# 6Lackiu/EMplanner_Carla

Measured on AMD Instinct MI355X. Metric: planning cycles/sec (DP+QP, 40x9 S-L lattice, 8 obs), higher is better.
Workload: dtype f64

## Files before the change

### emplanner_carla_amd/csrc/emp_frenet_core.h

```cpp
#pragma once

#include "emp_core.h"

namespace emp {

struct Node {
    double x, y, theta, kappa;
};
EMP_HD Node node_at(const double* line, int i) { return Node{line[4 * i], line[4 * i + 1], line[4 * i + 2], line[4 * i + 3]}; }

EMP_HD int match_scan(const double* line, int n_ref, double x, double y, int first, int step, int limit) {
    int match = 0, worse = 0;
    double best = __builtin_inf();
    for (int i = first; i >= 0 && i < n_ref; i += step) {
        const double dx = line[4 * i] - x, dy = line[4 * i + 1] - y;
        const double d = sqrt(dx * dx + dy * dy);
        if (d < best) {
            best = d;
            match = i;
            worse = 0;
        } else if (++worse >= limit) {
            break;
        }
    }
    return match;
}

EMP_HD double dot2(double a0, double a1, double b0, double b1) { return __builtin_fma(a1, b1, a0 * b0); }

EMP_HD Node project_on(const Node& m, double x, double y) {
    const double c = cos(m.theta), s = sin(m.theta);
    const double ds = dot2(x - m.x, y - m.y, c, s);
    return Node{m.x + ds * c, m.y + ds * s, m.theta + m.kappa * ds, m.kappa};
}

EMP_HD Node project_on_cs(const Node& m, double c, double s, double x, double y) {
    const double ds = dot2(x - m.x, y - m.y, c, s);
    return Node{m.x + ds * c, m.y + ds * s, m.theta + m.kappa * ds, m.kappa};
}
EMP_HD double projection_s_cs(const Node& m, double c, double s, double s_at_m, double x, double y) {
    return s_at_m + dot2(x - m.x, y - m.y, c, s);
}

EMP_HD double projection_s(const Node& m, double s_at_m, double x, double y) {
    return s_at_m + dot2(x - m.x, y - m.y, cos(m.theta), sin(m.theta));
}

EMP_HD double lateral_offset(const Node& proj, double x, double y) {
    return dot2(x - proj.x, y - proj.y, -sin(proj.theta), cos(proj.theta));
}

EMP_HD void s_map_build(const double* line, int n_ref, double ox, double oy, double* s_map) {
    const int m0 = match_scan(line, n_ref, ox, oy, 0, 1, 50);
    double acc = 0.0;
    s_map[0] = 0.0;
    for (int i = 1; i < n_ref; ++i) {
        const double dx = line[4 * i] - line[4 * (i - 1)], dy = line[4 * i + 1] - line[4 * (i - 1) + 1];
        acc = sqrt(dx * dx + dy * dy) + acc;
        s_map[i] = acc;
    }
    const double s0 = projection_s(node_at(line, m0), s_map[m0], ox, oy);
    for (int i = 0; i < n_ref; ++i) s_map[i] = s_map[i] - s0;
}

struct FrenetState {
    double l, l_dot, s_dot, l_ddot, dl_ds, s_ddot, ddl_ds;
};
EMP_HD FrenetState frenet_state(const Node& proj, double px, double py, double vx, double vy, double ax, double ay) {
    FrenetState o;
    const double c = cos(proj.theta), s = sin(proj.theta);
    const double k = proj.kappa;
    o.l = dot2(px - proj.x, py - proj.y, -s, c);
    o.l_dot = dot2(vx, vy, -s, c);
    o.s_dot = dot2(vx, vy, c, s) / (1.0 - k * o.l);
    o.l_ddot = dot2(ax, ay, -s, c) - k * (1.0 - k * o.l) * (o.s_dot * o.s_dot);
    o.dl_ds = (fabs(o.s_dot) < 1e-6) ? 0.0 : o.l_dot / o.s_dot;
    o.s_ddot = (dot2(ax, ay, c, s) + 2.0 * (o.s_dot * o.s_dot * k * o.dl_ds) + o.s_dot * o.s_dot * 0.0 * o.l) / (1.0 - k * o.l);
    o.ddl_ds = (fabs(o.s_dot) < 1e-6) ? 0.0 : (o.l_ddot - o.dl_ds * o.s_ddot) / (o.s_dot * o.s_dot);
    return o;
}

EMP_HD bool proj_point(const double* line, const double* s_map, int n_ref, double s, int* idx, Node* out) {
    int i = *idx;
    while (true) {
        if (i + 1 >= n_ref) return false;
        if (!(s_map[i + 1] < s)) break;
        ++i;
    }
    const Node m = node_at(line, i);
    const double ds = s - s_map[i];
    *out = Node{m.x + ds * cos(m.theta), m.y + ds * sin(m.theta), m.theta + m.kappa * ds, m.kappa};
    *idx = i;
    return true;
}

EMP_HD void heading_kappa(const double* xy, int stride, int m, double* theta, int tstride, double* kappa, int kstride) {
    for (int i = 0; i < m; ++i) {
        const int a = (i - 1 > 0) ? i - 1 : 0, b = (i < m - 2) ? i : m - 2;
        const double dx = ((xy[(a + 1) * stride] - xy[a * stride]) + (xy[(b + 1) * stride] - xy[b * stride])) / 2.0;
        const double dy = ((xy[(a + 1) * stride + 1] - xy[a * stride + 1]) + (xy[(b + 1) * stride + 1] - xy[b * stride + 1])) / 2.0;
        theta[i * tstride] = atan2(dy, dx);
    }
    for (int i = 0; i < m; ++i) {
        const int a = (i - 1 > 0) ? i - 1 : 0, b = (i < m - 2) ? i : m - 2;
        const double dx = ((xy[(a + 1) * stride] - xy[a * stride]) + (xy[(b + 1) * stride] - xy[b * stride])) / 2.0;
        const double dy = ((xy[(a + 1) * stride + 1] - xy[a * stride + 1]) + (xy[(b + 1) * stride + 1] - xy[b * stride + 1])) / 2.0;
        const double dpre = theta[(a + 1) * tstride] - theta[a * tstride];
        const double daft = theta[(b + 1) * tstride] - theta[b * tstride];
        kappa[i * kstride] = sin((dpre + daft) / 2.0) / sqrt(dx * dx + dy * dy);
    }
}

}
```

### emplanner_carla_amd/csrc/emp_tail_kernels.h

```cpp
#pragma once

#include <hip/hip_runtime.h>

#include "emp_core.h"
#include "emp_frenet_core.h"
#include "emp_qp_core.h"
#include "emp_qp_wave.h"
#include "emp_qp_rows.h"
#include "emp_smooth_rows.h"

namespace emp {

constexpr int kStDpInfeasible = 1, kStSOutOfRange = 2, kStBoundIndex = 4, kStQpFailed = 8, kStSmoothFailed = 16,
              kStTruncated = 32;

struct QpDev {
    PathQpParams qp;
    double obs_length, obs_width;
    int decimate, midpoint, use_qp;
    int debug_stage;
};

template <int CTRL, int ROW_MASK>
__device__ __forceinline__ void prefix_min_step(double& d, int& li) {
// ... 31 lines not shown
    const int lane = threadIdx.x & 63;
    double d = __builtin_inf();
    if (lane < P) {
        const double dx = lx[lane] - x, dy = ly[lane] - y;
        d = sqrt(dx * dx + dy * dy);
    }
    double pm = d;
    pm = prefix_fmin_step<0x111, 0xF>(pm);
    pm = prefix_fmin_step<0x112, 0xF>(pm);
    pm = prefix_fmin_step<0x114, 0xF>(pm);
    pm = prefix_fmin_step<0x118, 0xF>(pm);
    pm = prefix_fmin_step<0x142, 0xA>(pm);
    pm = prefix_fmin_step<0x143, 0xC>(pm);
    const double back = __shfl(pm, lane >= limit ? lane - limit : 0, 64);
    const unsigned long long stop = __ballot(lane < P && lane >= limit && pm == back);
    const int last = stop ? __builtin_ffsll((long long)stop) - 1 : P - 1;
    const double target = __shfl(pm, last, 64);
    const unsigned long long hit = __ballot(lane <= last && d == target);
    return hit ? __builtin_ffsll((long long)hit) - 1 : 0;
}

__device__ inline int match_scan_wave(const double* lx, const double* ly, int P, double x, double y, int limit) {
    if (P <= 64 && limit >= 1) return match_scan_wave64(lx, ly, P, x, y, limit);
    const int lane = threadIdx.x & 63;
    double cd = __builtin_inf();
    int ci = 0;
    for (int base = 0; base < P; base += 64) {
        const int i = base + lane;
        double d = __builtin_inf();
        int li = i;
        if (i < P) {
            const double dx = lx[i] - x, dy = ly[i] - y;
            d = sqrt(dx * dx + dy * dy);
        }
        prefix_min_first(d, li);
        if (!(d < cd)) {
            d = cd;
            li = ci;
        }
        const unsigned long long stop = __ballot(i < P && i - li >= limit);
        if (stop) {
            const int first = __builtin_ffsll((long long)stop) - 1;
            return __shfl(li, first, 64);
        }
        const int last = min(63, P - 1 - base);
        cd = __shfl(d, last, 64);
        ci = __shfl(li, last, 64);
    }
    return ci;
}

__global__ __launch_bounds__(64) void frenet_project_wave_kernel(
    int B, int max_ref, int max_obs, const double* __restrict__ ref_line, const int* __restrict__ n_ref,
    const double* __restrict__ origin_xy, const double* __restrict__ start_xy, const double* __restrict__ start_v,
    const double* __restrict__ start_a, const double* __restrict__ obs_xy, const int* __restrict__ n_obs,
    double* __restrict__ s_map, double* __restrict__ obs_s, double* __restrict__ obs_l, double* __restrict__ begin_sl,
    double* __restrict__ start, int obs_cap, const double* __restrict__ dyn, int* __restrict__ n_obs_out) {
    __builtin_amdgcn_s_setprio(EMP_PRIO_FRONT);
    extern __shared__ __attribute__((aligned(16))) double lds[];
    const int b = blockIdx.x, lane = threadIdx.x & 63;
    double* lx = lds;
    double* ly = lx + max_ref;
    double* lth = ly + max_ref;
    double* lk = lth + max_ref;
    double* sm = lk + max_ref;
    double* lcos = sm + max_ref;
    double* lsin = lcos + max_ref;
    const double* line = ref_line + (size_t)b * max_ref * 4;
    const int P = min(max(n_ref[b], 0), max_ref);
    const int k = n_obs ? min(max(n_obs[b], 0), max_obs) : 0;
    const double ox = origin_xy[2 * b], oy = origin_xy[2 * b + 1];
    const double px = start_xy[2 * b], py = start_xy[2 * b + 1];
    double obx = 0.0, oby = 0.0;
    if (lane < k) {
        obx = obs_xy[((size_t)b * max_obs + lane) * 2];
        oby = obs_xy[((size_t)b * max_obs + lane) * 2 + 1];
    }
    for (int i = lane; i < P; i += 64) {
        lx[i] = line[4 * i];
        ly[i] = line[4 * i + 1];
        const double th = line[4 * i + 2];
        lth[i] = th;
        lk[i] = line[4 * i + 3];
        lcos[i] = cos(th);
        lsin[i] = sin(th);
    }
    if (P == 0 && lane == 0) {
        lx[0] = ly[0] = lth[0] = lk[0] = sm[0] = lsin[0] = 0.0;
        lcos[0] = 1.0;
    }
    __syncthreads();
    double carry = 0.0;
    for (int base = 0; base < P; base += 64) {
        const int i = base + lane;
        double d = 0.0;
        if (i >= 1 && i < P) {
            const double dx = lx[i] - lx[i - 1], dy = ly[i] - ly[i - 1];
            d = sqrt(dx * dx + dy * dy);
        }
        const int cnt = min(64, P - base);
        if (lane == 0) d = (base >= 1) ? d + carry : 0.0;
        double mine = d;
        for (int k = 1; k < cnt; ++k) mine = d + lane_up1(mine);
        carry = __shfl(mine, cnt - 1, 64);
        if (i < P) sm[i] = mine;
    }
    __syncthreads();
    auto node = [&](int i) { return Node{lx[i], ly[i], lth[i], lk[i]}; };
    const int m0 = match_scan_wave(lx, ly, P, ox, oy, 50);
    const double s0 = projection_s_cs(node(m0), lcos[m0], lsin[m0], sm[m0], ox, oy);
    __syncthreads();
    for (int i = lane; i < P; i += 64) {
        const double v = sm[i] - s0;
        sm[i] = v;
        s_map[(size_t)b * max_ref + i] = v;
    }
    __syncthreads();
    int my_match = 0, first_match = 0;
    for (int j = 0; j < k; ++j) {
        if (j >= 64 && (j & 63) == 0 && (j & ~63) + lane < k) {
            obx = obs_xy[((size_t)b * max_obs + (j & ~63) + lane) * 2];
            oby = obs_xy[((size_t)b * max_obs + (j & ~63) + lane) * 2 + 1];
        }
        const double x = __shfl(obx, j & 63, 64), y = __shfl(oby, j & 63, 64);
        const int mj = match_scan_wave(lx, ly, P, x, y, 50);
        if (j == 0) first_match = mj;
        if ((j & 63) == lane) my_match = mj;
        if ((j & 63) == 63 || j == k - 1) {
            const int jj = (j & ~63) + lane;
            if (jj <= j) {
                obs_s[(size_t)b * obs_cap + jj] = projection_s_cs(node(my_match), lcos[my_match], lsin[my_match], sm[my_match], obx, oby);
                obs_l[(size_t)b * obs_cap + jj] = lateral_offset(project_on_cs(node(first_match), lcos[first_match], lsin[first_match], obx, oby), obx, oby);
            }
        }
    }
    const int ms = match_scan_wave(lx, ly, P, px, py, 50);
    if (lane == 0) {
        const Node proj = project_on_cs(node(ms), lcos[ms], lsin[ms], px, py);
        const double bs = projection_s_cs(node(ms), lcos[ms], lsin[ms], sm[ms], px, py);
        if (begin_sl) {
            begin_sl[2 * b] = bs;
            begin_sl[2 * b + 1] = lateral_offset(proj, px, py);
        }
        const FrenetState fs = frenet_state(proj, px, py, start_v[2 * b], start_v[2 * b + 1], start_a[2 * b], start_a[2 * b + 1]);
        start[4 * b + 0] = bs;
        start[4 * b + 1] = fs.l;
        start[4 * b + 2] = fs.dl_ds;
        start[4 * b + 3] = fs.ddl_ds;
        int total = k;
        if (dyn && !isnan(dyn[2 * b]) && k + 3 <= obs_cap) {
            const double Len_vehicle = 2.910, Len_obs = 3.0;
            const double Dis = dyn[2 * b], V_obs = dyn[2 * b + 1];
            const double vx = start_v[2 * b], vy = start_v[2 * b + 1];
            const double V_ego = sqrt(vx * vx + vy * vy);
            const double delta_v = V_ego - V_obs;
            const double meet_t = ((Dis - Len_vehicle / 2.0) - Len_obs / 2.0) / delta_v;
            const double delta_t = (Len_vehicle + Len_obs) / delta_v;
            const double leave_t = meet_t + delta_t;
            const double meet_s = ((bs + Dis) + V_obs * meet_t) - Len_obs / 2.0;
            const double leave_s = ((bs + Dis) + V_obs * leave_t) + Len_obs / 2.0;
            const double delta_s = leave_s - meet_s;
            const double obs_pos = meet_s + delta_s / 2.0;
            if (leave_s < 80.0) {
                double* os = obs_s + (size_t)b * obs_cap + k;
                double* ol = obs_l + (size_t)b * obs_cap + k;
                os[0] = meet_s - 10.0;
                os[1] = obs_pos;
                os[2] = leave_s;
                ol[0] = ol[1] = ol[2] = 0.0;
                total = k + 3;
            }
        }
        if (n_obs_out) n_obs_out[b] = total;
    }
}

__device__ inline int find_match_one(const double* line, int P, double x, double y, bool windowed, int st) {
    if (!windowed) return match_scan(line, P, x, y, 0, 1, 50);
    const Node pm = node_at(line, st);
    const double flag = dot2(x - pm.x, y - pm.y, cos(pm.theta), sin(pm.theta));
    return match_scan(line, P, x, y, st, flag > 0.0 ? 1 : -1, 5);
}

__global__ void match_points_kernel(int B, int max_ref, int max_pts, const double* __restrict__ ref_line,
                                    const int* __restrict__ n_ref, const double* __restrict__ xy,
                                    const int* __restrict__ n_pts, const int* __restrict__ is_first_run,
                                    const int* __restrict__ pre_match_index, int* __restrict__ match_index,
                                    double* __restrict__ proj, int windowed_api) {
    const int b = blockIdx.x * blockDim.x + threadIdx.x;
    if (b >= B) return;
    const double* line = ref_line + (size_t)b * max_ref * 4;
    const int P = min(max(n_ref[b], 0), max_ref);
    const int k = min(max(n_pts[b], 0), max_pts);
    int m_first = 0;
    const bool windowed = windowed_api && !is_first_run[b];
    if (P < 1 || (windowed && (pre_match_index[b] < 0 || pre_match_index[b] >= P))) {
        for (int j = 0; j < k; ++j) {
            match_index[(size_t)b * max_pts + j] = -1;
            double* o = proj + ((size_t)b * max_pts + j) * 4;
            o[0] = o[1] = o[2] = o[3] = __builtin_nan("");
        }
        return;
    }
    for (int j = 0; j < k; ++j) {
        const double x = xy[((size_t)b * max_pts + j) * 2], y = xy[((size_t)b * max_pts + j) * 2 + 1];
        const int m = find_match_one(line, P, x, y, windowed, windowed ? pre_match_index[b] : 0);
        if (j == 0) m_first = m;
        match_index[(size_t)b * max_pts + j] = m;
        const Node pr = project_on(node_at(line, m_first), x, y);
        double* o = proj + ((size_t)b * max_pts + j) * 4;
        o[0] = pr.x;
        o[1] = pr.y;
        o[2] = pr.theta;
        o[3] = pr.kappa;
    }
}

__global__ void heading_kappa_kernel(int B, int max_pts, const double* __restrict__ xy, const int* __restrict__ n_pts,
                                     double* __restrict__ theta, double* __restrict__ kappa) {
    const int b = blockIdx.x * blockDim.x + threadIdx.x;
    if (b >= B) return;
    const int m = min(max(n_pts[b], 0), max_pts);
    if (m < 2) return;
    heading_kappa(xy + (size_t)b * max_pts * 2, 2, m, theta + (size_t)b * max_pts, 1, kappa + (size_t)b * max_pts, 1);
}

__device__ inline int argmin_abs(const double* s, int stride, int n, double target) {
    int best = 0;
    double bv = fabs(s[0] - target);
    for (int j = 1; j < n; ++j) {
        const double v = fabs(s[j * stride] - target);
        if (v < bv) {
            bv = v;
            best = j;
        }
    }
    return best;
}

__device__ inline void argmin_abs3(const double* s, int n, double t0, double t1, double t2, int* i0, int* i1, int* i2) {
    const double f = s[0];
    double b0 = fabs(f - t0), b1 = fabs(f - t1), b2 = fabs(f - t2);
    int k0 = 0, k1 = 0, k2 = 0;
    for (int j0 = 1; j0 < n; j0 += 4) {
        double v[4];
#pragma unroll
        for (int u = 0; u < 4; ++u) v[u] = s[min(j0 + u, n - 1)];
#pragma unroll
        for (int u = 0; u < 4; ++u) {
            const int j = j0 + u;
            const double a0 = fabs(v[u] - t0), a1 = fabs(v[u] - t1), a2 = fabs(v[u] - t2);
            if (a0 < b0) { b0 = a0; k0 = j; }
            if (a1 < b1) { b1 = a1; k1 = j; }
            if (a2 < b2) { b2 = a2; k2 = j; }
        }
    }
// ... 101 lines not shown
        status[b] = rc ? kStSmoothFailed : 0;
    }
}

constexpr int kRefLinePoints = 51;

__global__ __launch_bounds__(64) void reference_line_wave_kernel(int B, int max_global, SmoothQpParams sx, SmoothQpParams sy,
                                                                 const double* __restrict__ global_path,
                                                                 const int* __restrict__ n_global,
                                                                 const double* __restrict__ pred_xy,
                                                                 const int* __restrict__ is_first_run,
                                                                 const int* __restrict__ pre_match_index,
                                                                 double* __restrict__ ref_line, int* __restrict__ n_ref,
                                                                 int* __restrict__ match_index, int* __restrict__ iters,
                                                                 int* __restrict__ status, int n_ref_on_fail = 0) {
    extern __shared__ __attribute__((aligned(16))) double lds[];
    const int b = blockIdx.x, lane = threadIdx.x & 63;
    const double* line = global_path + (size_t)b * max_global * 4;
    const int P = min(n_global[b], max_global);
    double* gxy = lds;
    double* qmem = gxy + 2 * kRefLinePoints;
    double* out = ref_line + (size_t)b * kRefLinePoints * 4;
    int m = 0, first = 0, fail = 0;
    if (lane == 0) {
        const double x = pred_xy[2 * b], y = pred_xy[2 * b + 1];
        const int st = pre_match_index[b];
        if (P < 1 || ((!is_first_run || !is_first_run[b]) && (st < 0 || st >= P))) {
            fail = kStSOutOfRange;
        } else if (is_first_run && is_first_run[b]) {
            m = match_scan(line, P, x, y, 0, 1, 50);
        } else {
            const Node pm = node_at(line, st);
            const double flag = dot2(x - pm.x, y - pm.y, cos(pm.theta), sin(pm.theta));
            m = match_scan(line, P, x, y, st, flag > 0.0 ? 1 : -1, 5);
        }
        int back = 10, fwd = 40;
        if (m < back) {
            back = m;
            fwd = 50 - back;
        }
        if (P - m - 1 < fwd) {
            fwd = P - m - 1;
            back = 50 - fwd;
        }
        first = m - back;
        if (!fail && (first < 0 || m + fwd + 1 > P)) fail = kStSOutOfRange;
    }
    m = __shfl(m, 0, 64);
    first = __shfl(first, 0, 64);
    fail = __shfl(fail, 0, 64);
    int it = 0;
    if (!fail) {
        if (lane < kRefLinePoints) {
            gxy[2 * lane] = line[4 * (first + lane)];
            gxy[2 * lane + 1] = line[4 * (first + lane) + 1];
        }
        __syncthreads();
        double *px = nullptr, *py = nullptr;
        const int rc = smooth_pair_wave<true>(qmem, gxy, 2, kRefLinePoints, sx, sy, &px, &py, &it);
        if (rc) fail = kStSmoothFailed;
        else heading_kappa_wave(px, py, kRefLinePoints, qmem + 2 * BoxRangeQp::words(kRefLinePoints, kRefLinePoints), out, 4);
    }
    if (fail)
        for (int i = lane; i < kRefLinePoints * 4; i += 64) out[i] = 0.0;
    if (lane == 0) {
        n_ref[b] = fail ? n_ref_on_fail : kRefLinePoints;
        match_index[b] = m;
        if (iters) iters[b] = it;
        status[b] = fail;
    }
}

__device__ inline int frenet_path_to_xy(const double* line, const double* s_map, int P, double begin_s, double begin_l,
                                        const double* path_s, const double* path_l, int n, double* target_xy,
                                        int cap, bool* s_error, bool* trunc) {
    *s_error = false;
    *trunc = false;
    int idx = 0, m = 0;
    Node pr;
    if (!proj_point(line, s_map, P, begin_s, &idx, &pr)) {
        *s_error = true;
        return 0;
    }
    target_xy[0] = pr.x + begin_l * (-sin(pr.theta));
    target_xy[1] = pr.y + begin_l * cos(pr.theta);
    m = 1;
    for (int i = 0; i < n; ++i) {
        const double s = path_s[i];
        if (s > s_map[P - 1]) break;
        if (!proj_point(line, s_map, P, s, &idx, &pr)) {
            *s_error = true;
            return m;
        }
        if (m >= cap) {
            *trunc = true;
            break;
        }
        target_xy[2 * m] = pr.x + path_l[i] * (-sin(pr.theta));
        target_xy[2 * m + 1] = pr.y + path_l[i] * cos(pr.theta);
        ++m;
    }
    return m;
}

__global__ void path_to_xy_kernel(int B, int max_ref, int max_pts, const double* __restrict__ ref_line,
                                  const double* __restrict__ s_map, const int* __restrict__ n_ref,
                                  const double* __restrict__ begin_sl, const double* __restrict__ path_s,
                                  const double* __restrict__ path_l, const int* __restrict__ n_pts,
                                  double* __restrict__ target_xy, int* __restrict__ n_out, int* __restrict__ status) {
    const int b = blockIdx.x * blockDim.x + threadIdx.x;
    if (b >= B) return;
    const int P = min(max(n_ref[b], 0), max_ref);
    const int n = min(max(n_pts[b], 0), max_pts);
    bool s_err, trunc;
    const int m = frenet_path_to_xy(ref_line + (size_t)b * max_ref * 4, s_map + (size_t)b * max_ref, P,
                                    begin_sl[2 * b], begin_sl[2 * b + 1], path_s + (size_t)b * max_pts,
                                    path_l + (size_t)b * max_pts, n, target_xy + (size_t)b * (max_pts + 1) * 2,
                                    max_pts + 1, &s_err, &trunc);
    n_out[b] = m;
    status[b] = (s_err ? kStSOutOfRange : 0) | (trunc ? kStTruncated : 0);
}

template <int G, int R = 0>
__host__ __device__ constexpr int cycle_qp_group_words(int cap, int max_obs) {
    if (R > 0) return PathQpRowsLayout<(R > 0 ? G : 8), (R > 0 ? R : 3)>::stride(max_obs);
    return 5 * cap + 4 * max_obs + (G == 32 ? path_qp_words_pair() : path_qp_words(cap));
}
template <int G, int R = 0>
__device__ __forceinline__ void cycle_qp_body(int B, int max_pts, int max_obs, int cap, const QpDev& Q,
                                                           const double* __restrict__ dp_s,
                                                           const double* __restrict__ dp_l,
                                                           const int* __restrict__ dp_len,
                                                           const double* __restrict__ obs_s,
                                                           const double* __restrict__ obs_l,
                                                           const int* __restrict__ n_obs,
                                                           const double* __restrict__ start,
                                                           double* __restrict__ path_s, double* __restrict__ path_l,
                                                           int* __restrict__ path_len, int* __restrict__ status) {
    extern __shared__ __attribute__((aligned(16))) double lds_all[];
    __builtin_amdgcn_s_setprio(EMP_PRIO_BACK);
    constexpr int GPW = 64 / G;
    const int lane = threadIdx.x & 63, grp = lane / G, gl = lane & (G - 1);
    const int b = blockIdx.x * GPW + grp;
    const bool present = b < B;
    static_assert(R == 0 || G == 8 || G == 16, "the rows solver runs on groups of 8 or 16 lanes");
    const int per_group = cycle_qp_group_words<G, R>(cap, max_obs);
    double* lds = lds_all + (size_t)grp * per_group;
    const size_t o = (size_t)(present ? b : 0) * max_pts;
    double* sd = lds;
    double *ld, *lmin, *lmax, *ql, *otab, *qmem;
    if constexpr (R > 0) {
        using L = PathQpRowsLayout<G, R>;
        qmem = lds;
        ql = qmem + L::result;
        sd = qmem + L::path;
        ld = sd + cap;
        lmin = ld + cap;
        lmax = lmin + cap;
        otab = qmem + (max_obs <= L::C ? L::obstacles : L::words);
    } else {
        ld = sd + cap;
        lmin = ld + cap;
        lmax = lmin + cap;
        ql = lmax + cap;
        otab = ql + cap;
        qmem = otab + 4 * max_obs;
    }
#ifdef EMP_QP_PROBE_EMPTY
    if (Q.debug_stage == 4) return;
#endif
    const int ne = present ? dp_len[b] : 0;
    const int dec = Q.decimate > 0 ? Q.decimate : 1;
    const int n = (ne + dec - 1) / dec;
    const int st = present ? status[b] : 0;
    int fail = 0;
    if (present && (n > cap || n + (Q.midpoint ? 1 : 0) > max_pts || n < 1)) fail = kStTruncated;
    bool live = present && !fail;
    for (int i = gl; i < (live ? n : 0); i += G) {
        sd[i] = dp_s[o + (size_t)i * dec];
        ld[i] = dp_l[o + (size_t)i * dec];
    }
    __syncthreads();
// ... 103 lines not shown
                    }
                }
                plen = n + 1;
            } else {
                for (int i = gl; i < n; i += G) {
                    ps[i] = sd_at(i);
                    pl[i] = ql[i];
                }
                plen = n;
            }
        }
        for (int i = plen + gl; i < max_pts; i += G) {
            ps[i] = 0.0;
            pl[i] = 0.0;
        }
        if (gl == 0) {
            path_len[b] = plen;
            status[b] = st | fail;
        }
    }
}

#define EMP_CYCLE_QP_PARAMS                                                                                         \
    int B, int max_pts, int max_obs, int cap, QpDev Q, const double *__restrict__ dp_s, const double *__restrict__ dp_l, \
        const int *__restrict__ dp_len, const double *__restrict__ obs_s, const double *__restrict__ obs_l,           \
        const int *__restrict__ n_obs, const double *__restrict__ start, double *__restrict__ path_s,                  \
        double *__restrict__ path_l, int *__restrict__ path_len, int *__restrict__ status
#define EMP_CYCLE_QP_ARGS B, max_pts, max_obs, cap, Q, dp_s, dp_l, dp_len, obs_s, obs_l, n_obs, start, path_s, path_l, path_len, status
template <int G>
__global__ __launch_bounds__(64) void cycle_qp_wave_kernel(EMP_CYCLE_QP_PARAMS) {
    cycle_qp_body<G>(EMP_CYCLE_QP_ARGS);
}
template <int GP, int R>
__global__ __launch_bounds__(64) void cycle_qp_rows_kernel(EMP_CYCLE_QP_PARAMS) {
    cycle_qp_body<GP, R>(EMP_CYCLE_QP_ARGS);
}
#undef EMP_CYCLE_QP_PARAMS
#undef EMP_CYCLE_QP_ARGS

__device__ inline int walk_from_zero(const double* sm, int P, double s, bool* off_end) {
    int lo = 0, hi = P - 1;
    while (lo < hi) {
        const int mid = (lo + hi) >> 1;
        if (sm[mid + 1] < s) lo = mid + 1;
        else hi = mid;
    }
    *off_end = lo + 1 >= P;
    return lo;
}

template <bool WIDE>
__device__ __forceinline__ void cycle_cartesian_body(
    int B, int max_ref, int max_pts, int cap, SmoothQpParams sx, SmoothQpParams sy, const double* __restrict__ ref_line,
    const double* __restrict__ s_map, const int* __restrict__ n_ref, const double* __restrict__ begin_sl,
    const double* __restrict__ path_s, const double* __restrict__ path_l, const int* __restrict__ path_len,
    double* __restrict__ traj, int* __restrict__ traj_len, int* __restrict__ status) {
    extern __shared__ __attribute__((aligned(16))) double lds[];
    __builtin_amdgcn_s_setprio(EMP_PRIO_CART);
    const int b = blockIdx.x, lane = threadIdx.x & 63;
    double* sm = lds;
    double* txy = sm + max_ref;
    double* th = txy + 2 * cap;
    double* qmem = th + cap;
    const int st = status[b];
    double* out_rows = traj + (size_t)b * (max_pts + 1) * 4;
    auto body = [&]() -> int {
    const double* line = ref_line + (size_t)b * max_ref * 4;
    const int P = min(max(n_ref[b], 0), max_ref);
    const int n = path_len[b];
    for (int i = lane; i < P; i += 64) sm[i] = s_map[(size_t)b * max_ref + i];
    __syncthreads();
    bool off = false;
    const double bs = begin_sl[2 * b], bl = begin_sl[2 * b + 1];
    const int idx0 = walk_from_zero(sm, P, bs, &off);
    if (off || P < 2) {
        if (lane == 0) status[b] = st | kStSOutOfRange;
        return 0;
    }
    if (st & (kStQpFailed | kStBoundIndex | kStTruncated)) return 0;
    if (lane == 0) {
        const Node m0 = node_at(line, idx0);
        const double ds = bs - sm[idx0];
        const double th0 = m0.theta + m0.kappa * ds;
        txy[0] = (m0.x + ds * cos(m0.theta)) + bl * (-sin(th0));
        txy[1] = (m0.y + ds * sin(m0.theta)) + bl * cos(th0);
    }
    const double s_last = sm[P - 1];
    int carry = idx0, count = n;
    for (int base = 0; base < n; base += 64) {
        const int i = base + lane;
        const bool in = i < n;
        const double s = in ? path_s[(size_t)b * max_pts + i] : 0.0;
        const int first_bad = __builtin_ffsll((long long)__ballot(in && s > s_last));
        if (first_bad) count = min(count, base + first_bad - 1);
        bool o2 = false;
        int k = in ? walk_from_zero(sm, P, fmin(s, s_last), &o2) : 0;
        for (int d = 1; d < 64; d <<= 1) {
            const int v = __shfl_up(k, d, 64);
            if (lane >= d) k = max(k, v);
        }
        k = max(k, carry);
        carry = __shfl(k, 63, 64);
        if (in && i < count && i + 1 < cap) {
            const Node mm = node_at(line, k);
            const double ds = s - sm[k];
            const double thp = mm.theta + mm.kappa * ds;
            const double l = path_l[(size_t)b * max_pts + i];
            txy[2 * (i + 1)] = (mm.x + ds * cos(mm.theta)) + l * (-sin(thp));
            txy[2 * (i + 1) + 1] = (mm.y + ds * sin(mm.theta)) + l * cos(thp);
        }
        if (first_bad) break;
    }
    const int m = count + 1;
    __syncthreads();
    if (m > cap || m > max_pts + 1) {
        if (lane == 0) status[b] = st | kStTruncated;
        return 0;
    }
    if (m < 2) {
        if (lane == 0) status[b] = st | kStSmoothFailed;
        return 0;
    }
    int it = 0;
    double *px = nullptr, *py = nullptr;
    const int rc = smooth_pair_wave<WIDE>(qmem, txy, 2, m, sx, sy, &px, &py, &it);
    if (rc) {
        if (lane == 0) status[b] = st | kStSmoothFailed;
        return 0;
    }
    heading_kappa_wave(px, py, m, th, out_rows, 4);
    return m;
    };
    const int m_out = body();
    for (int i = m_out * 4 + lane; i < (max_pts + 1) * 4; i += 64) out_rows[i] = 0.0;
    if (lane == 0) traj_len[b] = m_out;
}

#define EMP_CARTESIAN_ARGS B, max_ref, max_pts, cap, sx, sy, ref_line, s_map, n_ref, begin_sl, path_s, path_l, path_len, traj, traj_len, status
__global__ __launch_bounds__(64) void cycle_cartesian_wave_kernel_wide(
    int B, int max_ref, int max_pts, int cap, SmoothQpParams sx, SmoothQpParams sy, const double* __restrict__ ref_line,
    const double* __restrict__ s_map, const int* __restrict__ n_ref, const double* __restrict__ begin_sl,
    const double* __restrict__ path_s, const double* __restrict__ path_l, const int* __restrict__ path_len,
    double* __restrict__ traj, int* __restrict__ traj_len, int* __restrict__ status) {
    cycle_cartesian_body<true>(EMP_CARTESIAN_ARGS);
}
__global__ __launch_bounds__(64) __attribute__((amdgpu_waves_per_eu(4, 4))) void cycle_cartesian_wave_kernel_narrow(
    int B, int max_ref, int max_pts, int cap, SmoothQpParams sx, SmoothQpParams sy, const double* __restrict__ ref_line,
    const double* __restrict__ s_map, const int* __restrict__ n_ref, const double* __restrict__ begin_sl,
    const double* __restrict__ path_s, const double* __restrict__ path_l, const int* __restrict__ path_len,
    double* __restrict__ traj, int* __restrict__ traj_len, int* __restrict__ status) {
    cycle_cartesian_body<false>(EMP_CARTESIAN_ARGS);
}
#undef EMP_CARTESIAN_ARGS

template <int GP, int R>
__global__ __launch_bounds__(64) void cycle_cartesian_rows_kernel(
    int B, int max_ref, int max_pts, int cap, SmoothQpParams sx, SmoothQpParams sy, const double* __restrict__ ref_line,
    const double* __restrict__ s_map, const int* __restrict__ n_ref, const double* __restrict__ begin_sl,
    const double* __restrict__ path_s, const double* __restrict__ path_l, const int* __restrict__ path_len,
    double* __restrict__ traj, int* __restrict__ traj_len, int* __restrict__ status, int force_fallback) {
    extern __shared__ __attribute__((aligned(16))) double lds[];
    __builtin_amdgcn_s_setprio(EMP_PRIO_CART);
    constexpr int SL = 2 * GP, SPW = 64 / SL;
    const int lane = threadIdx.x & 63, sc = lane / SL, sl = lane & (SL - 1);
    const int b = blockIdx.x * SPW + sc;
    const bool present = b < B;
    const size_t bb = present ? (size_t)b : 0;
    const int per_scene = max_ref + 5 * cap;
    double* sm = lds + (size_t)sc * per_scene;
    double* txy = sm + max_ref;
    double* th = txy + 2 * cap;
    double* px = th + cap;
    double* py = px + cap;
    double* qmem = lds + (size_t)SPW * per_scene;
    const int st = present ? status[bb] : 0;
    int add = 0;
    bool alive = present && !(st & (kStQpFailed | kStBoundIndex | kStTruncated));
    const double* line = ref_line + bb * max_ref * 4;
    const int P = present ? min(max(n_ref[bb], 0), max_ref) : 0;
    const int n = alive ? path_len[bb] : 0;
    for (int i = sl; i < P; i += SL) sm[i] = s_map[bb * max_ref + i];
    __syncthreads();
    bool off = false;
    const double bs = present ? begin_sl[2 * bb] : 0.0, bl = alive ? begin_sl[2 * bb + 1] : 0.0;
    const int idx0 = walk_from_zero(sm, P, bs, &off);
    if (present && (off || P < 2)) {
        add = kStSOutOfRange;
        alive = false;
    }
    if (alive && sl == 0) {
        const Node m0 = node_at(line, idx0);
        const double ds = bs - sm[idx0];
        const double th0 = m0.theta + m0.kappa * ds;
        txy[0] = (m0.x + ds * cos(m0.theta)) + bl * (-sin(th0));
        txy[1] = (m0.y + ds * sin(m0.theta)) + bl * cos(th0);
    }
    const double s_last = alive ? sm[P - 1] : 0.0;
    int carry = idx0, count = alive ? n : 0;
    bool stop = !alive;
    int nmax = 0;
#pragma unroll
    for (int g = 0; g < SPW; ++g) nmax = max(nmax, __builtin_amdgcn_readlane(alive ? n : 0, SL * g));
    constexpr unsigned long long kSceneMask = (SL == 32) ? 0xffffffffull : 0xffffull;
    for (int base = 0; base < nmax; base += SL) {
        const int i = base + sl;
        const bool in = !stop && i < n;
        const double s = in ? path_s[bb * max_pts + i] : 0.0;
        const unsigned bad16 = (unsigned)((__ballot(in && s > s_last) >> (SL * sc)) & kSceneMask);
        const int first_bad = __builtin_ffs((int)bad16);
        if (!stop && first_bad) count = min(count, base + first_bad - 1);
        bool o2 = false;
        int k = in ? walk_from_zero(sm, P, fmin(s, s_last), &o2) : 0;
        for (int d = 1; d < SL; d <<= 1) {
            const int v = __shfl_up(k, d, SL);
            if (sl >= d) k = max(k, v);
        }
        k = max(k, carry);
        carry = __shfl(k, SL - 1, SL);
        if (in && i < count && i + 1 < cap) {
            const Node mm = node_at(line, k);
            const double ds = s - sm[k];
            const double thp = mm.theta + mm.kappa * ds;
            const double l = path_l[bb * max_pts + i];
            txy[2 * (i + 1)] = (mm.x + ds * cos(mm.theta)) + l * (-sin(thp));
            txy[2 * (i + 1) + 1] = (mm.y + ds * sin(mm.theta)) + l * cos(thp);
        }
        if (first_bad) stop = true;
    }
    int m = count + 1;
    __syncthreads();
    if (alive && (m > cap || m > max_pts + 1 || m > GP * R)) {
        add = kStTruncated;
        alive = false;
    }
    if (alive && m < 2) {
        add = kStSmoothFailed;
        alive = false;
    }
    const int grp = sl / GP, gl = sl & (GP - 1);
    double ref[R], u[R];
#pragma unroll
    for (int r = 0; r < R; ++r) {
        const int j = gl * R + r;
        const double v = txy[2 * (j < cap ? j : 0) + grp];
        ref[r] = (alive && j < m) ? v : 0.0;
    }
    int it = 0;
    int rc = box_qp_active_set_rows<GP, R>(ref, alive ? m : 0, grp ? sy : sx, u, &it);
    if (force_fallback && rc == 0) rc = -1;
    const unsigned long long unsettled = __ballot(alive && rc < 0), wrong = __ballot(alive && rc > 0);
    const bool need_fb = ((unsettled >> (SL * sc)) & kSceneMask) != 0ull;
    if (((wrong >> (SL * sc)) & kSceneMask) != 0ull) {
        add = kStSmoothFailed;
        alive = false;
    }
    if (alive && !need_fb) {
#pragma unroll
        for (int r = 0; r < R; ++r) {
            const int j = gl * R + r;
            if (j < m) (grp ? py : px)[j] = u[r];
        }
    }
    __syncthreads();
    if (unsettled != 0ull) {
        for (int s2 = 0; s2 < SPW; ++s2) {
            if (((unsettled >> (SL * s2)) & kSceneMask) == 0ull) continue;
            const int m2 = __builtin_amdgcn_readlane(m, SL * s2);
            double* base2 = lds + (size_t)s2 * per_scene;
            double *qx = nullptr, *qy = nullptr;
            int it2 = 0;
            const int rc2 = smooth_pair_wave<(GP * R > 32)>(qmem, base2 + max_ref, 2, m2, sx, sy, &qx, &qy, &it2);
            if (rc2 == 0) {
                for (int i = lane; i < m2; i += 64) {
                    base2[max_ref + 3 * cap + i] = qx[i];
                    base2[max_ref + 4 * cap + i] = qy[i];
                }
            } else if (sc == s2) {
                add = kStSmoothFailed;
                alive = false;
            }
            __syncthreads();
        }
    }
    double* out_rows = traj + bb * (max_pts + 1) * 4;
    const int mm = alive ? m : 0;
    for (int i = sl; i < mm; i += SL) {
        const int a = (i - 1 > 0) ? i - 1 : 0, c = (i < mm - 2) ? i : mm - 2;
        const double dx = ((px[a + 1] - px[a]) + (px[c + 1] - px[c])) / 2.0;
        const double dy = ((py[a + 1] - py[a]) + (py[c + 1] - py[c])) / 2.0;
        th[i] = atan2(dy, dx);
    }
    __syncthreads();
    for (int i = sl; i < mm; i += SL) {
        const int a = (i - 1 > 0) ? i - 1 : 0, c = (i < mm - 2) ? i : mm - 2;
        const double dx = ((px[a + 1] - px[a]) + (px[c + 1] - px[c])) / 2.0;
        const double dy = ((py[a + 1] - py[a]) + (py[c + 1] - py[c])) / 2.0;
        const double dpre = th[a + 1] - th[a], daft = th[c + 1] - th[c];
        double* o = out_rows + (size_t)i * 4;
        o[0] = px[i];
        o[1] = py[i];
        o[2] = th[i];
        o[3] = sin((dpre + daft) / 2.0) / sqrt(dx * dx + dy * dy);
    }
    if (present) {
        for (int i = mm * 4 + sl; i < (max_pts + 1) * 4; i += SL) out_rows[i] = 0.0;
        if (sl == 0) {
            traj_len[bb] = mm;
            if (add) status[bb] = st | add;
// ... 54 lines not shown
    int m_first = 0;
    for (int j = 0; j < k; ++j) {
        const size_t o = (size_t)b * max_pts + j;
        double* r = out + o * 7;
        if (P < 1) {
            r[0] = r[1] = r[2] = r[3] = r[4] = r[5] = r[6] = __builtin_nan("");
            continue;
        }
        const double x = xy[o * 2], y = xy[o * 2 + 1];
        const int m = match_scan(line, P, x, y, 0, 1, 50);
        if (j == 0) m_first = m;
        const Node proj = project_on(node_at(line, m_first), x, y);
        const FrenetState f = frenet_state(proj, origin_xy[2 * b], origin_xy[2 * b + 1], vxy[o * 2], vxy[o * 2 + 1],
                                           axy[o * 2], axy[o * 2 + 1]);
        r[0] = f.l; r[1] = f.l_dot; r[2] = f.s_dot; r[3] = f.l_ddot; r[4] = f.dl_ds; r[5] = f.s_ddot; r[6] = f.ddl_ds;
    }
}

__global__ void proj_point_kernel(int n, int max_ref, const double* __restrict__ ref_line,
                                  const double* __restrict__ s_map, const int* __restrict__ n_ref,
                                  const double* __restrict__ s, const int* __restrict__ pre_idx,
                                  double* __restrict__ out, int* __restrict__ idx_out, int* __restrict__ status) {
    const int t = blockIdx.x * blockDim.x + threadIdx.x;
    if (t >= n) return;
    const int P = min(max(n_ref[t], 0), max_ref);
    int idx = pre_idx[t];
    Node pr{0, 0, 0, 0};
    const bool ok = idx >= 0 && proj_point(ref_line + (size_t)t * max_ref * 4, s_map + (size_t)t * max_ref, P, s[t], &idx, &pr);
    out[4 * t] = pr.x; out[4 * t + 1] = pr.y; out[4 * t + 2] = pr.theta; out[4 * t + 3] = pr.kappa;
    idx_out[t] = idx;
    status[t] = ok ? 0 : kStSOutOfRange;
}

__device__ inline double chord_length(double x0, double y0, double x1, double y1) {
    const double dx = x1 - x0, dy = y1 - y0;
    return sqrt(dx * dx + dy * dy);
}

__global__ void index2s_kernel(int B, int max_pts, const double* __restrict__ x, const double* __restrict__ y,
                               const int* __restrict__ n_pts, double* __restrict__ out) {
    const int b = blockIdx.x * blockDim.x + threadIdx.x;
    if (b >= B) return;
    const size_t o = (size_t)b * max_pts;
    const int n = min(max(n_pts[b], 0), max_pts);
    double acc = 0.0;
    for (int i = 0; i < n; ++i) out[o + i] = 0.0;
    for (int i = 1; i < n; ++i) {
        if (x[o + i] != x[o + i]) break;
        acc += chord_length(x[o + i - 1], y[o + i - 1], x[o + i], y[o + i]);
        out[o + i] = acc;
    }
}

__global__ void frenet2cartesian_kernel(int B, int max_ref, int max_pts, const double* __restrict__ ref_line,
                                        const double* __restrict__ index2s, const int* __restrict__ n_ref,
                                        const double* __restrict__ sl, const int* __restrict__ n_pts,
                                        double* __restrict__ out, int* __restrict__ status, int proj_only) {
    const int b = blockIdx.x * blockDim.x + threadIdx.x;
    if (b >= B) return;
    const double* line = ref_line + (size_t)b * max_ref * 4;
    const double* sm = index2s + (size_t)b * max_ref;
    const int P = min(max(n_ref[b], 0), max_ref);
    const int k = min(max(n_pts[b], 0), max_pts);
    const double qnan = __builtin_nan("");
    int st = 0;
    bool stopped = false;
    for (int j = 0; j < k; ++j) {
        const double* v = sl + ((size_t)b * max_pts + j) * 4;
        double* o = out + ((size_t)b * max_pts + j) * 4;
        o[0] = o[1] = o[2] = o[3] = qnan;
        if (stopped || v[0] != v[0]) {
            stopped = true;
            continue;
        }
        int idx = 1;
        while (idx < P && sm[idx] < v[0]) ++idx;
        if (idx >= P) {
            st = kStSOutOfRange;
            stopped = true;
            continue;
        }
        const Node m = node_at(line, idx);
        const double ds = v[0] - sm[idx];
        const double px = m.x + ds * cos(m.theta), py = m.y + ds * sin(m.theta);
        const double ph = m.theta + ds * m.kappa, pk = m.kappa;
        if (proj_only) {
            o[0] = px; o[1] = py; o[2] = ph; o[3] = pk;
            continue;
        }
        const double l = v[1], dl = v[2], ddl = v[3];
        o[0] = px + l * (-sin(ph));
        o[1] = py + l * cos(ph);
        const double hd = ph + atan(dl / (1.0 - pk * l));
        const double dth = hd - ph;
        o[2] = hd;
        o[3] = ((ddl + pk * dl * tan(dth)) * (cos(dth) * cos(dth)) / (1.0 - pk * l) + pk) * cos(dth) / (1.0 - pk * l);
    }
    status[b] = st;
}

__device__ inline void dy_obs_deri_one(double l, double vx, double vy, double hd, double k, double* s_dot_out, double* l_dot_out,
                                       double* dl_out) {
    const double l_dot = dot2(vx, vy, -sin(hd), cos(hd));
    const double s_dot = dot2(vx, vy, cos(hd), sin(hd)) / (1.0 - k * l);
    *s_dot_out = s_dot;
    *l_dot_out = l_dot;
    *dl_out = (fabs(s_dot) < 1e-6) ? 0.0 : l_dot / s_dot;
}

__global__ void dy_obs_deri_kernel(int n, const double* __restrict__ in, double* __restrict__ out) {
    const int t = blockIdx.x * blockDim.x + threadIdx.x;
    if (t >= n) return;
    dy_obs_deri_one(in[5 * t], in[5 * t + 1], in[5 * t + 2], in[5 * t + 3], in[5 * t + 4], &out[3 * t], &out[3 * t + 1], &out[3 * t + 2]);
}

__global__ void quintic_kernel(int n, const double* __restrict__ bc, double* __restrict__ coeff) {
    const int t = blockIdx.x * blockDim.x + threadIdx.x;
    if (t >= n) return;
    const double* v = bc + 8 * t;
    const double l0 = v[0], dl0 = v[1], ddl0 = v[2], l1 = v[3], dl1 = v[4], ddl1 = v[5], s0 = v[6], T = v[7] - v[6];
    const double h = l1 - l0, T2 = T * T, T3 = T2 * T, T4 = T3 * T, T5 = T4 * T;
    double a[6];
    a[0] = l0;
    a[1] = dl0;
    a[2] = 0.5 * ddl0;
    a[3] = (20.0 * h - (8.0 * dl1 + 12.0 * dl0) * T - (3.0 * ddl0 - ddl1) * T2) / (2.0 * T3);
    a[4] = (-30.0 * h + (14.0 * dl1 + 16.0 * dl0) * T + (3.0 * ddl0 - 2.0 * ddl1) * T2) / (2.0 * T4);
    a[5] = (12.0 * h - 6.0 * (dl1 + dl0) * T - (ddl0 - ddl1) * T2) / (2.0 * T5);
    double c[6] = {a[5], 0, 0, 0, 0, 0};
    int deg = 0;
    for (int k = 4; k >= 0; --k) {
        ++deg;
        for (int j = deg; j >= 1; --j) c[j] = c[j - 1] - s0 * c[j];
        c[0] = a[k] - s0 * c[0];
    }
    for (int j = 0; j < 6; ++j) coeff[6 * t + j] = c[j];
}

__global__ void obs_cost_kernel(int n, int samples, double w, double danger, double safe, const double* __restrict__ sq,
                                double* __restrict__ cost) {
    const int t = blockIdx.x * blockDim.x + threadIdx.x;
    if (t >= n) return;
    const double d2a = danger * danger, d2b = safe * safe;
    double c = 0.0;
    for (int i = 0; i < samples; ++i) {
        const double v = sq[(size_t)samples * t + i];
        if (v <= d2a) {
            c = c + w;
            break;
        } else if (d2a < v && v < d2b) {
            c = c + kSoftGain / v;
        }
    }
    cost[t] = c;
}

__global__ void free_edge_cost_kernel(int n, int max_obs, const double* __restrict__ edges, const double* __restrict__ obs_s,
                                      const double* __restrict__ obs_l, const int* __restrict__ n_obs, double w_coll, double w0,
                                      double w1, double w2, double w_ref, double* __restrict__ cost) {
    const int t = blockIdx.x * blockDim.x + threadIdx.x;
    if (t >= n) return;
    const double* e = edges + (size_t)t * 8;
    const Quintic q = quintic_shifted(e[1], e[2], e[3], e[5], e[4]);
    const int k = max_obs > 0 ? min(max(n_obs[t], 0), max_obs) : 0;
    cost[t] = segment_cost(q, e[0], e[6], obs_s + (size_t)t * max_obs, obs_l + (size_t)t * max_obs, k, w_coll, w0, w1, w2, w_ref);
}

}
```

Baseline: 18.45 million.

## Fuse sin/cos into sincos and fold serial start-point work into lane-parallel loops

Replaces separate sin and cos calls on the same angle with a combined sincos on the device, so argument reduction is shared. The start-point projection and Frenet state, previously computed serially by lane 0 after the obstacle loop, now run as an extra slot in the obstacle batch. The first trajectory point in the wave-parallel smoothing kernel is produced by lane q==0 inside the main loop instead of a separate serial block. This removes serial tail work and redundant transcendental evaluations, at the cost of more complex index bookkeeping (count offset by 2, q=i+1).

After: 18.64 million (median of 6 runs). +1.0%, better.

```diff
diff --git a/emplanner_carla_amd/csrc/emp_frenet_core.h b/emplanner_carla_amd/csrc/emp_frenet_core.h
--- a/emplanner_carla_amd/csrc/emp_frenet_core.h
+++ b/emplanner_carla_amd/csrc/emp_frenet_core.h
@@ -28,8 +28,18 @@
 
 EMP_HD double dot2(double a0, double a1, double b0, double b1) { return __builtin_fma(a1, b1, a0 * b0); }
 
+EMP_HD void sincos_pair(double x, double* s, double* c) {
+#if defined(__HIP_DEVICE_COMPILE__)
+    sincos(x, s, c);
+#else
+    *s = sin(x);
+    *c = cos(x);
+#endif
+}
+
 EMP_HD Node project_on(const Node& m, double x, double y) {
-    const double c = cos(m.theta), s = sin(m.theta);
+    double c, s;
+    sincos_pair(m.theta, &s, &c);
     const double ds = dot2(x - m.x, y - m.y, c, s);
     return Node{m.x + ds * c, m.y + ds * s, m.theta + m.kappa * ds, m.kappa};
 }
@@ -43,11 +53,18 @@
 }
 
 EMP_HD double projection_s(const Node& m, double s_at_m, double x, double y) {
-    return s_at_m + dot2(x - m.x, y - m.y, cos(m.theta), sin(m.theta));
+    double c, sn;
+    sincos_pair(m.theta, &sn, &c);
+    return s_at_m + dot2(x - m.x, y - m.y, c, sn);
 }
 
 EMP_HD double lateral_offset(const Node& proj, double x, double y) {
-    return dot2(x - proj.x, y - proj.y, -sin(proj.theta), cos(proj.theta));
+    double c, s;
+    sincos_pair(proj.theta, &s, &c);
+    return dot2(x - proj.x, y - proj.y, -s, c);
+}
+EMP_HD double lateral_offset_cs(const Node& proj, double c, double s, double x, double y) {
+    return dot2(x - proj.x, y - proj.y, -s, c);
 }
 
 EMP_HD void s_map_build(const double* line, int n_ref, double ox, double oy, double* s_map) {
@@ -66,9 +83,9 @@
 struct FrenetState {
     double l, l_dot, s_dot, l_ddot, dl_ds, s_ddot, ddl_ds;
 };
-EMP_HD FrenetState frenet_state(const Node& proj, double px, double py, double vx, double vy, double ax, double ay) {
+EMP_HD FrenetState frenet_state_cs(const Node& proj, double c, double s, double px, double py, double vx, double vy, double ax,
+                                   double ay) {
     FrenetState o;
-    const double c = cos(proj.theta), s = sin(proj.theta);
     const double k = proj.kappa;
     o.l = dot2(px - proj.x, py - proj.y, -s, c);
     o.l_dot = dot2(vx, vy, -s, c);
@@ -78,6 +95,11 @@
     o.s_ddot = (dot2(ax, ay, c, s) + 2.0 * (o.s_dot * o.s_dot * k * o.dl_ds) + o.s_dot * o.s_dot * 0.0 * o.l) / (1.0 - k * o.l);
     o.ddl_ds = (fabs(o.s_dot) < 1e-6) ? 0.0 : (o.l_ddot - o.dl_ds * o.s_ddot) / (o.s_dot * o.s_dot);
     return o;
+}
+EMP_HD FrenetState frenet_state(const Node& proj, double px, double py, double vx, double vy, double ax, double ay) {
+    double c, s;
+    sincos_pair(proj.theta, &s, &c);
+    return frenet_state_cs(proj, c, s, px, py, vx, vy, ax, ay);
 }
 
 EMP_HD bool proj_point(const double* line, const double* s_map, int n_ref, double s, int* idx, Node* out) {
@@ -89,7 +111,9 @@
     }
     const Node m = node_at(line, i);
     const double ds = s - s_map[i];
-    *out = Node{m.x + ds * cos(m.theta), m.y + ds * sin(m.theta), m.theta + m.kappa * ds, m.kappa};
+    double c, sn;
+    sincos_pair(m.theta, &sn, &c);
+    *out = Node{m.x + ds * c, m.y + ds * sn, m.theta + m.kappa * ds, m.kappa};
     *idx = i;
     return true;
 }
diff --git a/emplanner_carla_amd/csrc/emp_tail_kernels.h b/emplanner_carla_amd/csrc/emp_tail_kernels.h
--- a/emplanner_carla_amd/csrc/emp_tail_kernels.h
+++ b/emplanner_carla_amd/csrc/emp_tail_kernels.h
@@ -137,8 +137,10 @@
         const double th = line[4 * i + 2];
         lth[i] = th;
         lk[i] = line[4 * i + 3];
-        lcos[i] = cos(th);
-        lsin[i] = sin(th);
+        double sn, cs;
+        sincos_pair(th, &sn, &cs);
+        lcos[i] = cs;
+        lsin[i] = sn;
     }
     if (P == 0 && lane == 0) {
         lx[0] = ly[0] = lth[0] = lk[0] = sm[0] = lsin[0] = 0.0;
@@ -171,33 +173,12 @@
         s_map[(size_t)b * max_ref + i] = v;
     }
     __syncthreads();
-    int my_match = 0, first_match = 0;
-    for (int j = 0; j < k; ++j) {
-        if (j >= 64 && (j & 63) == 0 && (j & ~63) + lane < k) {
-            obx = obs_xy[((size_t)b * max_obs + (j & ~63) + lane) * 2];
-            oby = obs_xy[((size_t)b * max_obs + (j & ~63) + lane) * 2 + 1];
-        }
-        const double x = __shfl(obx, j & 63, 64), y = __shfl(oby, j & 63, 64);
-        const int mj = match_scan_wave(lx, ly, P, x, y, 50);
-        if (j == 0) first_match = mj;
-        if ((j & 63) == lane) my_match = mj;
-        if ((j & 63) == 63 || j == k - 1) {
-            const int jj = (j & ~63) + lane;
-            if (jj <= j) {
-                obs_s[(size_t)b * obs_cap + jj] = projection_s_cs(node(my_match), lcos[my_match], lsin[my_match], sm[my_match], obx, oby);
-                obs_l[(size_t)b * obs_cap + jj] = lateral_offset(project_on_cs(node(first_match), lcos[first_match], lsin[first_match], obx, oby), obx, oby);
-            }
-        }
-    }
-    const int ms = match_scan_wave(lx, ly, P, px, py, 50);
-    if (lane == 0) {
-        const Node proj = project_on_cs(node(ms), lcos[ms], lsin[ms], px, py);
-        const double bs = projection_s_cs(node(ms), lcos[ms], lsin[ms], sm[ms], px, py);
+    auto planning_start = [&](double bs, double l, const Node& proj, double pc, double psn) {
         if (begin_sl) {
             begin_sl[2 * b] = bs;
-            begin_sl[2 * b + 1] = lateral_offset(proj, px, py);
-        }
-        const FrenetState fs = frenet_state(proj, px, py, start_v[2 * b], start_v[2 * b + 1], start_a[2 * b], start_a[2 * b + 1]);
+            begin_sl[2 * b + 1] = l;
+        }
+        const FrenetState fs = frenet_state_cs(proj, pc, psn, px, py, start_v[2 * b], start_v[2 * b + 1], start_a[2 * b], start_a[2 * b + 1]);
         start[4 * b + 0] = bs;
         start[4 * b + 1] = fs.l;
         start[4 * b + 2] = fs.dl_ds;
@@ -227,6 +208,38 @@
             }
         }
         if (n_obs_out) n_obs_out[b] = total;
+    };
+    const int ms = match_scan_wave(lx, ly, P, px, py, 50);
+    int my_match = 0, first_match = 0;
+    for (int j = 0; j <= k; ++j) {
+        if (j < k) {
+            if (j >= 64 && (j & 63) == 0 && (j & ~63) + lane < k) {
+                obx = obs_xy[((size_t)b * max_obs + (j & ~63) + lane) * 2];
+                oby = obs_xy[((size_t)b * max_obs + (j & ~63) + lane) * 2 + 1];
+            }
+            const double x = __shfl(obx, j & 63, 64), y = __shfl(oby, j & 63, 64);
+            const int mj = match_scan_wave(lx, ly, P, x, y, 50);
+            if (j == 0) first_match = mj;
+            if ((j & 63) == lane) my_match = mj;
+        }
+        if ((j & 63) != 63 && j != k) continue;
+        const int jj = (j & ~63) + lane;
+        const bool is_start = jj == k;
+        if (jj <= j) {
+            const int m_s = is_start ? ms : my_match, m_l = is_start ? ms : first_match;
+            const double x = is_start ? px : obx, y = is_start ? py : oby;
+            const double bs = projection_s_cs(node(m_s), lcos[m_s], lsin[m_s], sm[m_s], x, y);
+            const Node proj = project_on_cs(node(m_l), lcos[m_l], lsin[m_l], x, y);
+            double pc, psn;
+            sincos_pair(proj.theta, &psn, &pc);
+            const double l = lateral_offset_cs(proj, pc, psn, x, y);
+            if (!is_start) {
+                obs_s[(size_t)b * obs_cap + jj] = bs;
+                obs_l[(size_t)b * obs_cap + jj] = l;
+            } else {
+                planning_start(bs, l, proj, pc, psn);
+            }
+        }
     }
 }
 
@@ -494,8 +507,10 @@
         *s_error = true;
         return 0;
     }
-    target_xy[0] = pr.x + begin_l * (-sin(pr.theta));
-    target_xy[1] = pr.y + begin_l * cos(pr.theta);
+    double pc, psn;
+    sincos_pair(pr.theta, &psn, &pc);
+    target_xy[0] = pr.x + begin_l * (-psn);
+    target_xy[1] = pr.y + begin_l * pc;
     m = 1;
     for (int i = 0; i < n; ++i) {
         const double s = path_s[i];
@@ -508,8 +523,9 @@
             *trunc = true;
             break;
         }
-        target_xy[2 * m] = pr.x + path_l[i] * (-sin(pr.theta));
-        target_xy[2 * m + 1] = pr.y + path_l[i] * cos(pr.theta);
+        sincos_pair(pr.theta, &psn, &pc);
+        target_xy[2 * m] = pr.x + path_l[i] * (-psn);
+        target_xy[2 * m + 1] = pr.y + path_l[i] * pc;
         ++m;
     }
     return m;
@@ -779,8 +795,11 @@
         const Node m0 = node_at(line, idx0);
         const double ds = bs - sm[idx0];
         const double th0 = m0.theta + m0.kappa * ds;
-        txy[0] = (m0.x + ds * cos(m0.theta)) + bl * (-sin(th0));
-        txy[1] = (m0.y + ds * sin(m0.theta)) + bl * cos(th0);
+        double mc, msn, pc, psn;
+        sincos_pair(m0.theta, &msn, &mc);
+        sincos_pair(th0, &psn, &pc);
+        txy[0] = (m0.x + ds * mc) + bl * (-psn);
+        txy[1] = (m0.y + ds * msn) + bl * pc;
     }
     const double s_last = sm[P - 1];
     int carry = idx0, count = n;
@@ -803,8 +822,11 @@
             const double ds = s - sm[k];
             const double thp = mm.theta + mm.kappa * ds;
             const double l = path_l[(size_t)b * max_pts + i];
-            txy[2 * (i + 1)] = (mm.x + ds * cos(mm.theta)) + l * (-sin(thp));
-            txy[2 * (i + 1) + 1] = (mm.y + ds * sin(mm.theta)) + l * cos(thp);
+            double mc, msn, pc, psn;
+            sincos_pair(mm.theta, &msn, &mc);
+            sincos_pair(thp, &psn, &pc);
+            txy[2 * (i + 1)] = (mm.x + ds * mc) + l * (-psn);
+            txy[2 * (i + 1) + 1] = (mm.y + ds * msn) + l * pc;
         }
         if (first_bad) break;
     }
@@ -885,27 +907,21 @@
         add = kStSOutOfRange;
         alive = false;
     }
-    if (alive && sl == 0) {
-        const Node m0 = node_at(line, idx0);
-        const double ds = bs - sm[idx0];
-        const double th0 = m0.theta + m0.kappa * ds;
-        txy[0] = (m0.x + ds * cos(m0.theta)) + bl * (-sin(th0));
-        txy[1] = (m0.y + ds * sin(m0.theta)) + bl * cos(th0);
-    }
     const double s_last = alive ? sm[P - 1] : 0.0;
     int carry = idx0, count = alive ? n : 0;
     bool stop = !alive;
-    int nmax = 0;
+    int qmax = 0;
 #pragma unroll
-    for (int g = 0; g < SPW; ++g) nmax = max(nmax, __builtin_amdgcn_readlane(alive ? n : 0, SL * g));
+    for (int g = 0; g < SPW; ++g) qmax = max(qmax, __builtin_amdgcn_readlane(alive ? n + 1 : 0, SL * g));
     constexpr unsigned long long kSceneMask = (SL == 32) ? 0xffffffffull : 0xffffull;
-    for (int base = 0; base < nmax; base += SL) {
-        const int i = base + sl;
-        const bool in = !stop && i < n;
+    for (int base = 0; base < qmax; base += SL) {
+        const int q = base + sl, i = q - 1;
+        const bool is0 = alive && q == 0;
+        const bool in = !stop && i >= 0 && i < n;
         const double s = in ? path_s[bb * max_pts + i] : 0.0;
         const unsigned bad16 = (unsigned)((__ballot(in && s > s_last) >> (SL * sc)) & kSceneMask);
         const int first_bad = __builtin_ffs((int)bad16);
-        if (!stop && first_bad) count = min(count, base + first_bad - 1);
+        if (!stop && first_bad) count = min(count, base + first_bad - 2);
         bool o2 = false;
         int k = in ? walk_from_zero(sm, P, fmin(s, s_last), &o2) : 0;
         for (int d = 1; d < SL; d <<= 1) {
@@ -914,13 +930,16 @@
         }
         k = max(k, carry);
         carry = __shfl(k, SL - 1, SL);
-        if (in && i < count && i + 1 < cap) {
+        if (is0 || (in && i < count && i + 1 < cap)) {
             const Node mm = node_at(line, k);
-            const double ds = s - sm[k];
+            const double ds = (is0 ? bs : s) - sm[k];
             const double thp = mm.theta + mm.kappa * ds;
-            const double l = path_l[bb * max_pts + i];
-            txy[2 * (i + 1)] = (mm.x + ds * cos(mm.theta)) + l * (-sin(thp));
-            txy[2 * (i + 1) + 1] = (mm.y + ds * sin(mm.theta)) + l * cos(thp);
+            const double l = is0 ? bl : path_l[bb * max_pts + i];
+            double mc, msn, pc, psn;
+            sincos_pair(mm.theta, &msn, &mc);
+            sincos_pair(thp, &psn, &pc);
+            txy[2 * q] = (mm.x + ds * mc) + l * (-psn);
+            txy[2 * q + 1] = (mm.y + ds * msn) + l * pc;
         }
         if (first_bad) stop = true;
     }
@@ -1141,15 +1160,19 @@
         }
         const Node m = node_at(line, idx);
         const double ds = v[0] - sm[idx];
-        const double px = m.x + ds * cos(m.theta), py = m.y + ds * sin(m.theta);
+        double mc, msn;
+        sincos_pair(m.theta, &msn, &mc);
+        const double px = m.x + ds * mc, py = m.y + ds * msn;
         const double ph = m.theta + ds * m.kappa, pk = m.kappa;
         if (proj_only) {
             o[0] = px; o[1] = py; o[2] = ph; o[3] = pk;
             continue;
         }
         const double l = v[1], dl = v[2], ddl = v[3];
-        o[0] = px + l * (-sin(ph));
-        o[1] = py + l * cos(ph);
+        double pc, psn;
+        sincos_pair(ph, &psn, &pc);
+        o[0] = px + l * (-psn);
+        o[1] = py + l * pc;
         const double hd = ph + atan(dl / (1.0 - pk * l));
         const double dth = hd - ph;
         o[2] = hd;
```
